# GlassyWing/yolo_deepsort

Measured on AMD Instinct MI355X. Metric: end-to-end frames/sec (detect+ReID+assoc), 608x608, higher is better.
Workload: dtype f16x3

## Files before the change

yolo_deepsort_amd/csrc/conv_block1.hip:

```cpp
#include "conv_common.h"

#include <algorithm>

namespace yds {

namespace {

constexpr int TH = 8, TW = 16;
constexpr int BM = TH * TW, BN = 64, WM = 4, WN = 2, NW = 8, NT = NW * 64;
constexpr int PR = TH + 2, PC = TW + 2, PPIX = PR * PC;
constexpr int CMID = 32, CIN = 64, GIN = CIN / 32;
constexpr int W3_BYTES = 9 * BN * 128, XP_BYTES = GIN * PPIX * 128, HP_BYTES = PPIX * 128;
constexpr int SMEM = W3_BYTES + XP_BYTES + HP_BYTES;
constexpr int XCHUNKS = GIN * PPIX * 8, XLOADS = (XCHUNKS + NT - 1) / NT;

struct PatchRows {
    int img, oy0, ox0, H, W;
    __device__ __forceinline__ int operator()(int row) const {
        const int oy = oy0 + row / TW, ox = ox0 + row % TW;
        return oy < H && ox < W ? (img * H + oy) * W + ox : -1;
    }
};

template <int ACT, bool HALF>
__global__ __launch_bounds__(NT, 1) void conv_block1_f16x3(ConvKernelArgs p2, ConvKernelArgs p3, int tiles_y, int tiles_x, int n_tiles) {
    fp16_saturate_on();
    extern __shared__ __attribute__((aligned(16))) char smem[];
    char *w3 = smem, *xp = smem + W3_BYTES, *hp = smem + W3_BYTES + XP_BYTES;
    const int tid = threadIdx.x, lane = tid & 63, wave = tid >> 6, wm = wave / WN, wn = wave % WN, kb = lane >> 5;
    const int H = p2.H, W = p2.W;

    for (int i = tid; i < 9 * BN * 8; i += NT) {
        const int row = i >> 3, pos = i & 7, tap = row / BN, co = row - tap * BN;
        const int c = pos ^ ((row >> 1) & 7);
        *reinterpret_cast<f32x4 *>(w3 + row * 128 + pos * 16) =
            *reinterpret_cast<const f32x4 *>(reinterpret_cast<const char *>(p3.w) + ((size_t)co * 9 + tap) * 128 + c * 16);
    }
    h8 w2h[4], w2l[4];
#pragma unroll
    for (int sb = 0; sb < 4; ++sb) {
        const char *g = reinterpret_cast<const char *>(p2.w) + ((size_t)(lane & 31) * GIN + (sb >> 1)) * 128;
        w2h[sb] = *reinterpret_cast<const h8 *>(g + (2 * (sb & 1) + kb) * 16);
        w2l[sb] = *reinterpret_cast<const h8 *>(g + 64 + (2 * (sb & 1) + kb) * 16);
    }
    float bias2[16];
#pragma unroll
    for (int e = 0; e < 16; ++e) bias2[e] = p2.bias[(e & 3) + 8 * (e >> 2) + 4 * kb] * A_SCALE;
    const int r = wm * 32 + (lane & 31), py = r / TW, px = r - py * TW;
    const int brow = wn * 32 + (lane & 31);

    const bool xs = p2.fmt_x == FMT_F16;
    f32x4 nxt[XLOADS];
    auto fetch = [&](int tl) {
        const int img = tl / (tiles_y * tiles_x), rem = tl - img * (tiles_y * tiles_x);
        const int iy0 = (rem / tiles_x) * TH - 1, ix0 = (rem % tiles_x) * TW - 1;
#pragma unroll
        for (int l = 0; l < XLOADS; ++l) {
            const int i = tid + l * NT, c = i & 7, row = i >> 3, g = row / PPIX, pr = row - g * PPIX;
            const int iy = iy0 + pr / PC, ix = ix0 + pr % PC;
            nxt[l] = f32x4{0.f, 0.f, 0.f, 0.f};
            if (i < XCHUNKS && tl < n_tiles && (unsigned)iy < (unsigned)H && (unsigned)ix < (unsigned)W && !(xs && c >= 4))
                nxt[l] = *reinterpret_cast<const f32x4 *>(reinterpret_cast<const char *>(p2.x + ((size_t)(img * H + iy) * W + ix) * p2.ldx) +
                                                          (xs ? (g * 4 + c) * 16 : g * 128 + c * 16));
        }
    };
    fetch(blockIdx.x);
    for (int tl = blockIdx.x; tl < n_tiles; tl += gridDim.x) {
        const int img = tl / (tiles_y * tiles_x), rem = tl - img * (tiles_y * tiles_x);
        const int oy0 = (rem / tiles_x) * TH, ox0 = (rem % tiles_x) * TW;
        __syncthreads();
#pragma unroll
        for (int l = 0; l < XLOADS; ++l) {
            const int i = tid + l * NT, c = i & 7, row = i >> 3;
            if (i < XCHUNKS) *reinterpret_cast<f32x4 *>(xp + row * 128 + ((c ^ ((row >> 1) & 7)) << 4)) = nxt[l];
        }
        __syncthreads();
        fetch(tl + gridDim.x);
        if (wave < (PPIX + 31) / 32) {
            const int pix = wave * 32 + (lane & 31), pr = min(pix, PPIX - 1);
            f32x16 c1, c2;
#pragma unroll
            for (int e = 0; e < 16; ++e) { c1[e] = 0.f; c2[e] = 0.f; }
#pragma unroll
            for (int sb = 0; sb < 4; ++sb) {
                const int row = (sb >> 1) * PPIX + pr, sw = (row >> 1) & 7;
                const char *ap = xp + row * 128;
                const h8 xh = *reinterpret_cast<const h8 *>(ap + (((2 * (sb & 1) + kb) ^ sw) << 4));
                c1 = __builtin_amdgcn_mfma_f32_32x32x16_f16(w2h[sb], xh, c1, 0, 0, 0);
                if (!HALF) {
                    const h8 xl = *reinterpret_cast<const h8 *>(ap + (((4 + 2 * (sb & 1) + kb) ^ sw) << 4));
                    c2 = __builtin_amdgcn_mfma_f32_32x32x16_f16(w2h[sb], xl, c2, 0, 0, 0);
                    c2 = __builtin_amdgcn_mfma_f32_32x32x16_f16(w2l[sb], xh, c2, 0, 0, 0);
                }
            }
            const int ry = pr / PC, rc = pr - ry * PC;
            const bool inside = (unsigned)(oy0 - 1 + ry) < (unsigned)H && (unsigned)(ox0 - 1 + rc) < (unsigned)W;
            const int sw = (pr >> 1) & 7;
            if (pix < PPIX) {
                if (inside) {
#pragma unroll
                    for (int g = 0; g < 4; ++g) {
                        float v[4];
#pragma unroll
                        for (int c = 0; c < 4; ++c) {
                            const int e = g * 4 + c;
                            const float os = (HALF ? c1[e] : c1[e] + c2[e] * (1.f / LO_SCALE)) + bias2[e];
                            v[c] = ACT == ACT_LEAKY ? fmaxf(os, os * 0.1f) : apply_act<ACT>(os * (1.f / A_SCALE)) * A_SCALE;
                        }
                        h16x4 hi, lo;
                        if (HALF) {
#pragma unroll
                            for (int c = 0; c < 4; ++c) hi[c] = (_Float16)v[c];
                        } else {
                            h16_encode4_scaled(v, hi, lo);
                        }
                        *reinterpret_cast<h16x4 *>(hp + pr * 128 + ((g ^ sw) << 4) + kb * 8) = hi;
                        if (!HALF) *reinterpret_cast<h16x4 *>(hp + pr * 128 + (((4 + g) ^ sw) << 4) + kb * 8) = lo;
                    }
                } else {
                    const h16x4 z = {(_Float16)0.f, (_Float16)0.f, (_Float16)0.f, (_Float16)0.f};
#pragma unroll
                    for (int g = 0; g < (HALF ? 4 : 8); ++g) *reinterpret_cast<h16x4 *>(hp + pr * 128 + ((g ^ sw) << 4) + kb * 8) = z;
                }
            }
        }
        __syncthreads();
        f32x16 acc1[1][1], acc2[1][1];
#pragma unroll
        for (int e = 0; e < 16; ++e) { acc1[0][0][e] = 0.f; acc2[0][0][e] = 0.f; }
#pragma unroll
        for (int t = 0; t < 9; ++t) {
            const int j = (py + t / 3) * PC + px + t % 3;
            const int jsw = (j >> 1) & 7, wrow = t * BN + brow, wsw = (wrow >> 1) & 7;
            const char *ap = hp + j * 128, *bp = w3 + wrow * 128;
#pragma unroll
            for (int s = 0; s < 2; ++s) {
                const h8 ah = *reinterpret_cast<const h8 *>(ap + (((2 * s + kb) ^ jsw) << 4));
                const h8 bh = *reinterpret_cast<const h8 *>(bp + (((2 * s + kb) ^ wsw) << 4));
                acc1[0][0] = __builtin_amdgcn_mfma_f32_32x32x16_f16(ah, bh, acc1[0][0], 0, 0, 0);
                if (!HALF) {
                    const h8 al = *reinterpret_cast<const h8 *>(ap + (((4 + 2 * s + kb) ^ jsw) << 4));
                    const h8 bl = *reinterpret_cast<const h8 *>(bp + (((4 + 2 * s + kb) ^ wsw) << 4));
                    acc2[0][0] = __builtin_amdgcn_mfma_f32_32x32x16_f16(ah, bl, acc2[0][0], 0, 0, 0);
                    acc2[0][0] = __builtin_amdgcn_mfma_f32_32x32x16_f16(al, bh, acc2[0][0], 0, 0, 0);
                }
            }
        }
#pragma unroll
        for (int e = 0; e < 16; ++e) acc1[0][0][e] = (HALF ? acc1[0][0][e] : acc1[0][0][e] + acc2[0][0][e] * (1.f / LO_SCALE)) * (1.f / A_SCALE);
        conv_epilogue_rows<BM, BN, WM, WN, ACT, RES_AFTER_ACT, 1, 1, NT, PatchRows, true>(p3, acc1, reinterpret_cast<float *>(xp),
                                                                                           PatchRows{img, oy0, ox0, H, W}, 0, tid);
    }
}

template <int ACT, bool HALF> void launch_inst(const ConvKernelArgs &k2, const ConvKernelArgs &k3, hipStream_t s) {
    static_assert(BM * (BN + 4) * 4 <= XP_BYTES, "whole-tile epilogue staging must fit the input patch");
    const int n_img = k2.M / (k2.H * k2.W);
    const int tiles_y = (k2.H + TH - 1) / TH, tiles_x = (k2.W + TW - 1) / TW, n_tiles = n_img * tiles_y * tiles_x;
    static bool attr_set = false;
    auto kern = conv_block1_f16x3<ACT, HALF>;
    if (!attr_set) {
        YDS_HIP(hipFuncSetAttribute(reinterpret_cast<const void *>(kern), hipFuncAttributeMaxDynamicSharedMemorySize, SMEM));
        attr_set = true;
    }
    hipLaunchKernelGGL(kern, dim3(std::min(n_tiles, 256)), dim3(NT), SMEM, s, k2, k3, tiles_y, tiles_x, n_tiles);
    YDS_HIP(hipGetLastError());
}

}

bool conv_block1_applicable(const ConvKernelArgs &k2, const ConvKernelArgs &k3) {
    return k2.Cin == CIN && k2.ksize == 1 && k2.stride == 1 && k2.Cout == CMID && k2.res_mode == RES_NONE && (k2.fmt_x == FMT_H16 || k2.fmt_x == FMT_F16) &&
           k3.Cin == CMID && k3.ksize == 3 && k3.stride == 1 && k3.pad == 1 && k3.Cout == BN && k3.res_mode == RES_AFTER_ACT &&
           k3.fmt_r == k2.fmt_x && k3.fmt_y == k2.fmt_x && k3.res == k2.x && k3.ldr == k2.ldx && k3.H == k2.H && k3.W == k2.W &&
           k2.act == k3.act && (k2.act == ACT_LEAKY || k2.act == ACT_MISH);
}

void launch_conv_block1(const ConvKernelArgs &k2, const ConvKernelArgs &k3, hipStream_t s) {
    if (!conv_block1_applicable(k2, k3)) fail("conv: the fused residual block takes conv1x1 64->32 + conv3x3 32->64 + shortcut to the block input");
    const bool half = k3.terms == 1;
    if (k2.act == ACT_LEAKY) { if (half) launch_inst<ACT_LEAKY, true>(k2, k3, s); else launch_inst<ACT_LEAKY, false>(k2, k3, s); }
    else { if (half) launch_inst<ACT_MISH, true>(k2, k3, s); else launch_inst<ACT_MISH, false>(k2, k3, s); }
}

}
```

yolo_deepsort_amd/csrc/conv_common.h:

```cpp
#pragma once
#include "common.h"
#include "h16.h"

#include <algorithm>
#include <stdlib.h>
#include <type_traits>

namespace yds {

typedef float f32x16 __attribute__((ext_vector_type(16)));
typedef float f32x4 __attribute__((ext_vector_type(4)));

typedef _Float16 h8 __attribute__((ext_vector_type(8)));
typedef _Float16 h4 __attribute__((ext_vector_type(4)));
constexpr float A_SCALE = 1.f / 256.f, LO_SCALE = 2048.f;
typedef __attribute__((address_space(3))) void lds_void_t;
typedef __attribute__((address_space(1))) const void glb_void_t;
template <int N> __device__ __forceinline__ void wait_vmcnt() { asm volatile("s_waitcnt vmcnt(%0)" ::"n"(N) : "memory"); }

struct ConvKernelArgs {
    const float *x, *w, *bias, *res;
    float *y;
    int H, W, Cin, ldx;
    int Ho, Wo, Cout, ldy, ldr;
    int ksize, stride, pad;
    int K, Kpad, M;
    int act, res_mode;
    int fmt_x, fmt_y, fmt_r;
    int terms;
    int ksplit = 1;
    float *y2 = nullptr;
    int ldy2 = 0, n_split = 0;
    int tiles_m, tiles_n, xm, rm, rn;
    int gn = 1;
    int gn_req = 0;
};

constexpr int KALIGN = 32;
constexpr int STAGGER = 24;

template <int ACT> __device__ __forceinline__ float apply_act(float v) {
    if (ACT == ACT_LEAKY) return v > 0.f ? v : v * 0.1f;
    if (ACT == ACT_RELU) return v > 0.f ? v : 0.f;
    if (ACT == ACT_MISH) {
        const float e = __builtin_amdgcn_exp2f(fminf(v, 20.f) * 1.44269504088896341f);
        const float n = e * (e + 2.f);
        const float m = v * (n * __builtin_amdgcn_rcpf(n + 2.f));
        return v > 20.f ? v : m;
    }
    return v;
}

__device__ __forceinline__ bool tile_of_block(const ConvKernelArgs &p, int &tm, int &tn) {
    const int b = blockIdx.x, xcd = b & 7, idx = b >> 3;
    int lm, ln;
    if (p.gn <= 1) {
        lm = idx % p.rm;
        ln = idx / p.rm;
    } else {
        const int per = p.rm * p.gn, grp = idx / per, w = idx - grp * per;
        const int g = min(p.gn, p.rn - grp * p.gn);
        lm = w / g;
        ln = grp * p.gn + (w - lm * g);
    }
    tm = (xcd % p.xm) * p.rm + lm;
    tn = (xcd / p.xm) * p.rn + ln;
    return tm < p.tiles_m && tn < p.tiles_n;
}

inline int plan_tile_map(ConvKernelArgs &k, int BM, int BN) {
    k.tiles_m = (k.M + BM - 1) / BM;
    k.tiles_n = (k.Cout + BN - 1) / BN;
    long best = -1;
    for (int xm = 1; xm <= 8; xm *= 2) {
        int xn = 8 / xm;
        int rm = (k.tiles_m + xm - 1) / xm, rn = (k.tiles_n + xn - 1) / xn;
        long waste = (long)rm * rn * 8 - (long)k.tiles_m * k.tiles_n;
        long cost = ((long)rm * BM + (long)rn * BN) * 64 + waste * (BM + BN);
        if (best < 0 || cost < best) { best = cost; k.xm = xm; k.rm = rm; k.rn = rn; }
    }
    k.gn = std::max(1, std::min(k.gn_req, k.rn));
    return 8 * k.rm * k.rn;
}

struct FlatRows {
    int m0;
    __device__ __forceinline__ int operator()(int row) const { return m0 + row; }
};
template <int BM, int BN, int WM, int WN, int ACT, int RES, int NT, class RowMap, bool ONE_PASS, class Store>
__device__ __forceinline__ void conv_epilogue_core(const ConvKernelArgs &p, Store store, float *stage, RowMap rows, int n0, int tid) {
    constexpr int ROWS = BM / WM, LD = BN + 4, C4 = BN / 4;
    constexpr int RSTEP = NT / C4;
    static_assert(NT % C4 == 0 && C4 % 2 == 0 && ROWS % RSTEP == 0, "tile width must divide the workgroup; lane pairs share a row");
    const int wave = tid >> 6, wm = wave / WN;
    const int c4 = tid % C4, rr = tid / C4;
    const int n = n0 + c4 * 4;
    const bool n_vec = n + 3 < p.Cout;
    const bool second = p.n_split > 0 && n >= p.n_split;
    float *const y_base = second ? p.y2 : p.y;
    const int y_ld = second ? p.ldy2 : p.ldy, ny = second ? n - p.n_split : n;
    float4 bias4 = make_float4(0.f, 0.f, 0.f, 0.f);
    if (n_vec) bias4 = *reinterpret_cast<const float4 *>(p.bias + n);
    else {
        if (n < p.Cout) bias4.x = p.bias[n];
        if (n + 1 < p.Cout) bias4.y = p.bias[n + 1];
        if (n + 2 < p.Cout) bias4.z = p.bias[n + 2];
    }
    constexpr int PER_PASS = ROWS / RSTEP, NRES = RES != RES_NONE ? WM * PER_PASS : 1;
    auto sweep = [&](auto yf_c, auto rf_c) {
        constexpr int YF = decltype(yf_c)::value, RF = decltype(rf_c)::value;
        constexpr bool YH = YF == FMT_H16, RH = RF == FMT_H16, YS = YF == FMT_F16, RS = RF == FMT_F16;
        float4 rraw[NRES];
        if (RES != RES_NONE) {
#pragma unroll
            for (int q = 0; q < NRES; ++q) {
                const int m = rows((q / PER_PASS) * ROWS + rr + (q % PER_PASS) * RSTEP);
                rraw[q] = make_float4(0.f, 0.f, 0.f, 0.f);
                if (m >= 0 && m < p.M && n < p.Cout) {
                    const float *rp = p.res + (size_t)m * p.ldr;
                    if (RH) {
                        const char *g = reinterpret_cast<const char *>(rp + (n & ~31)) + (n & 31) * 2;
                        const float2 hi = *reinterpret_cast<const float2 *>(g), lo = *reinterpret_cast<const float2 *>(g + 64);
                        rraw[q] = make_float4(hi.x, hi.y, lo.x, lo.y);
                    } else if (RS) {
                        const float2 h = *reinterpret_cast<const float2 *>(reinterpret_cast<const char *>(rp) + n * 2);
                        rraw[q] = make_float4(h.x, h.y, 0.f, 0.f);
                    } else if (n_vec) {
                        rraw[q] = *reinterpret_cast<const float4 *>(rp + n);
                    } else {
                        rraw[q].x = rp[n];
                        if (n + 1 < p.Cout) rraw[q].y = rp[n + 1];
                        if (n + 2 < p.Cout) rraw[q].z = rp[n + 2];
                    }
                }
            }
        }
#pragma unroll
        for (int pass = 0; pass < WM; ++pass) {
            if (ONE_PASS ? pass == 0 : wm == pass) store(stage + (ONE_PASS ? wm * ROWS * LD : 0));
            if (!ONE_PASS || pass == 0) __syncthreads();
#pragma unroll
            for (int k2 = 0; k2 < PER_PASS; ++k2) {
                const int r = rr + k2 * RSTEP;
                const int m = rows(pass * ROWS + r);
                const bool live = m >= 0 && m < p.M && n < p.Cout;
                float4 v = *reinterpret_cast<const float4 *>(stage + (ONE_PASS ? pass * ROWS * LD : 0) + r * LD + c4 * 4);
                float rs[4] = {0.f, 0.f, 0.f, 0.f};
                if (RES != RES_NONE) {
                    const float4 t = rraw[RES != RES_NONE ? pass * PER_PASS + k2 : 0];
                    if (RH) {
                        union { float2 f; h16x4 h; } uh, ul;
                        uh.f = make_float2(t.x, t.y);
                        ul.f = make_float2(t.z, t.w);
                        h16_decode4(uh.h, ul.h, rs);
                    } else if (RS) {
                        union { float2 f; h16x4 h; } uh;
                        uh.f = make_float2(t.x, t.y);
#pragma unroll
                        for (int k = 0; k < 4; ++k) rs[k] = (float)uh.h[k] * (1.f / H16_A_SCALE);
                    } else { rs[0] = t.x; rs[1] = t.y; rs[2] = t.z; rs[3] = t.w; }
                }
                float o[4] = {v.x + bias4.x, v.y + bias4.y, v.z + bias4.z, v.w + bias4.w};
#pragma unroll
                for (int k = 0; k < 4; ++k) {
                    if (RES == RES_BEFORE_ACT) o[k] += rs[k];
                    o[k] = apply_act<ACT>(o[k]);
                    if (RES == RES_AFTER_ACT) o[k] += rs[k];
                }
                float *yp = y_base + (size_t)m * y_ld;
                if (YH) {
                    h16x4 hi, lo;
                    h16_encode4(o, hi, lo);
                    const bool odd = c4 & 1;
                    union { h16x4 h; int i[2]; } send, recv;
                    send.h = odd ? hi : lo;
                    recv.i[0] = __builtin_amdgcn_update_dpp(send.i[0], send.i[0], 0xB1, 0xF, 0xF, false);
                    recv.i[1] = __builtin_amdgcn_update_dpp(send.i[1], send.i[1], 0xB1, 0xF, 0xF, false);
                    union { h16x4 h[2]; float4 f; } out;
                    out.h[0] = odd ? recv.h : hi;
                    out.h[1] = odd ? lo : recv.h;
                    const int nq = ny & ~7;
                    char *g = reinterpret_cast<char *>(yp + (nq & ~31)) + (nq & 31) * 2 + (odd ? 64 : 0);
                    if (live) *reinterpret_cast<float4 *>(g) = out.f;
                } else if (YS) {
                    union { h16x4 h; int i[2]; } mine, other;
#pragma unroll
                    for (int k = 0; k < 4; ++k) mine.h[k] = (_Float16)(o[k] * H16_A_SCALE);
                    other.i[0] = __builtin_amdgcn_update_dpp(mine.i[0], mine.i[0], 0xB1, 0xF, 0xF, false);
                    other.i[1] = __builtin_amdgcn_update_dpp(mine.i[1], mine.i[1], 0xB1, 0xF, 0xF, false);
                    union { h16x4 h[2]; float4 f; } out;
                    out.h[0] = mine.h;
                    out.h[1] = other.h;
                    if (live && !(c4 & 1)) *reinterpret_cast<float4 *>(reinterpret_cast<char *>(yp) + ny * 2) = out.f;
                } else if (live) {
                    if (n_vec) *reinterpret_cast<float4 *>(yp + ny) = make_float4(o[0], o[1], o[2], o[3]);
                    else { yp[ny] = o[0]; if (n + 1 < p.Cout) yp[ny + 1] = o[1]; if (n + 2 < p.Cout) yp[ny + 2] = o[2]; }
                }
            }
            if (!ONE_PASS && pass + 1 < WM) __syncthreads();
        }
    };
    using F32c = std::integral_constant<int, FMT_F32>;
    using H16c = std::integral_constant<int, FMT_H16>;
    using F16c = std::integral_constant<int, FMT_F16>;
    const bool yh = p.fmt_y == FMT_H16, rh = RES != RES_NONE && p.fmt_r == FMT_H16;
    if (p.fmt_y == FMT_F16) {
        sweep(F16c{}, F16c{});
    } else if (yh) {
        if (rh) sweep(H16c{}, H16c{});
        else sweep(H16c{}, F32c{});
    } else {
        if (rh) sweep(F32c{}, H16c{});
        else sweep(F32c{}, F32c{});
    }
}
constexpr size_t conv_stage_bytes(int BM, int BN) { return (size_t)BM * (BN + 4) * sizeof(float); }

template <int BM, int BN, int WM, int WN, int ACT, int RES, int TM, int TN, int NT = 256, class RowMap = FlatRows, bool ONE_PASS = false>
__device__ __forceinline__ void conv_epilogue_rows(const ConvKernelArgs &p, f32x16 (&acc)[TM][TN], float *stage, RowMap rows, int n0, int tid) {
    constexpr int LD = BN + 4;
    const int lane = tid & 63, wn = (tid >> 6) % WN;
    const int col = lane & 31, rsel = (lane >> 5) * 4;
    auto store = [&](float *st) {
#pragma unroll
        for (int i = 0; i < TM; ++i)
#pragma unroll
            for (int j = 0; j < TN; ++j)
#pragma unroll
                for (int e = 0; e < 16; ++e)
                    st[(i * 32 + rsel + (e & 3) + 8 * (e >> 2)) * LD + wn * (BN / WN) + j * 32 + col] = acc[i][j][e];
    };
    conv_epilogue_core<BM, BN, WM, WN, ACT, RES, NT, RowMap, ONE_PASS>(p, store, stage, rows, n0, tid);
}

template <int BM, int BN, int WM, int WN, int ACT, int RES, int TM, int TN, int NT = 256, class RowMap = FlatRows, bool ONE_PASS = false>
__device__ __forceinline__ void conv_epilogue16_rows(const ConvKernelArgs &p, f32x4 (&acc)[TM][TN], float *stage, RowMap rows, int n0, int tid) {
    constexpr int LD = BN + 4;
    const int lane = tid & 63, wn = (tid >> 6) % WN;
    const int col = lane & 15, rsel = (lane >> 4) * 4;
    auto store = [&](float *st) {
#pragma unroll
        for (int i = 0; i < TM; ++i)
#pragma unroll
            for (int j = 0; j < TN; ++j)
#pragma unroll
                for (int e = 0; e < 4; ++e)
                    st[(i * 16 + rsel + e) * LD + wn * (BN / WN) + j * 16 + col] = acc[i][j][e];
    };
    conv_epilogue_core<BM, BN, WM, WN, ACT, RES, NT, RowMap, ONE_PASS>(p, store, stage, rows, n0, tid);
}
template <int BM, int BN, int WM, int WN, int ACT, int RES, int TM, int TN, int NT = 256, bool ONE_PASS = false>
__device__ __forceinline__ void conv_epilogue16(const ConvKernelArgs &p, f32x4 (&acc)[TM][TN], float *stage, int m0, int n0, int tid) {
    conv_epilogue16_rows<BM, BN, WM, WN, ACT, RES, TM, TN, NT, FlatRows, ONE_PASS>(p, acc, stage, FlatRows{m0}, n0, tid);
}

template <int BM, int BN, int WM, int WN, int ACT, int RES, int TM, int TN, int NT = 256, bool ONE_PASS = false>
__device__ __forceinline__ void conv_epilogue(const ConvKernelArgs &p, f32x16 (&acc)[TM][TN], float *stage, int m0, int n0, int tid) {
    conv_epilogue_rows<BM, BN, WM, WN, ACT, RES, TM, TN, NT, FlatRows, ONE_PASS>(p, acc, stage, FlatRows{m0}, n0, tid);
}

ConvKernelArgs make_conv_args(const ConvArgs &a);
bool conv_stem2_applicable(const ConvKernelArgs &k0, const ConvKernelArgs &k1);
void launch_conv_stem2(const ConvKernelArgs &k0, const ConvKernelArgs &k1, hipStream_t s);
bool conv_block1_applicable(const ConvKernelArgs &k2, const ConvKernelArgs &k3);
void launch_conv_block1(const ConvKernelArgs &k2, const ConvKernelArgs &k3, hipStream_t s);

template <class F> void dispatch_act_res(const ConvKernelArgs &k, F f) {
    using Linear = std::integral_constant<int, ACT_LINEAR>;
    using Leaky = std::integral_constant<int, ACT_LEAKY>;
    using Mish = std::integral_constant<int, ACT_MISH>;
    using Relu = std::integral_constant<int, ACT_RELU>;
    using None = std::integral_constant<int, RES_NONE>;
    using After = std::integral_constant<int, RES_AFTER_ACT>;
    using Before = std::integral_constant<int, RES_BEFORE_ACT>;
    switch (k.act * 4 + k.res_mode) {
        case ACT_LINEAR * 4 + RES_NONE: f(Linear{}, None{}); break;
        case ACT_LEAKY * 4 + RES_NONE: f(Leaky{}, None{}); break;
        case ACT_LEAKY * 4 + RES_AFTER_ACT: f(Leaky{}, After{}); break;
        case ACT_MISH * 4 + RES_NONE: f(Mish{}, None{}); break;
        case ACT_MISH * 4 + RES_AFTER_ACT: f(Mish{}, After{}); break;
        case ACT_RELU * 4 + RES_NONE: f(Relu{}, None{}); break;
        case ACT_RELU * 4 + RES_BEFORE_ACT: f(Relu{}, Before{}); break;
        default: fail("conv: unsupported activation/residual combination (%d, %d)", k.act, k.res_mode);
    }
}

template <auto KERN, class... Args>
void launch_conv_tiles(ConvKernelArgs k, int BM, int BN, int grid_y, int threads, size_t smem, hipStream_t s, Args... args) {
    static size_t attr_set = 0;
    if (smem > attr_set) {
        YDS_HIP(hipFuncSetAttribute(reinterpret_cast<const void *>(KERN), hipFuncAttributeMaxDynamicSharedMemorySize, (int)smem));
        attr_set = smem;
    }
    dim3 grid(plan_tile_map(k, BM, BN), grid_y);
    hipLaunchKernelGGL(KERN, grid, dim3(threads), smem, s, k, args...);
    YDS_HIP(hipGetLastError());
}

bool conv_direct_applicable(const ConvKernelArgs &k);
void launch_conv_direct(const ConvKernelArgs &k, hipStream_t s);
bool conv_pool_applicable(const ConvKernelArgs &k);
void launch_conv_pool(const ConvKernelArgs &k, hipStream_t s);

void launch_conv_f16x3_staged(ConvKernelArgs k, int tile, hipStream_t s);
void launch_conv_f16x3_dma(ConvKernelArgs k, int tile, hipStream_t s);
void launch_conv_f16x3_win(ConvKernelArgs k, int tile, hipStream_t s);
void launch_conv_f16x3_splitk(ConvKernelArgs k, int tile, hipStream_t s);
bool conv_splitk_applicable(const ConvKernelArgs &k, int tile);
bool conv_splitk_preferred(const ConvKernelArgs &k);
bool conv_win2_applicable(const ConvKernelArgs &k);
void launch_conv_win2(ConvKernelArgs k, hipStream_t s);
bool conv_win_applicable(const ConvKernelArgs &k);
void launch_conv_win(ConvKernelArgs k, int shape, hipStream_t s);
void conv_win_clock(unsigned long long *cycles_ticks, bool reset);
void conv_win16_clock(unsigned long long *cycles_ticks, bool reset);
bool conv_win16_small_applicable(const ConvKernelArgs &k);
void launch_conv_win16(ConvKernelArgs k, int shape, hipStream_t s);
void conv_win2_clock(unsigned long long *cycles_ticks, bool reset);

}
```

yolo_deepsort_amd/csrc/conv_stem2.hip:

```cpp
#include "conv_common.h"

#include <algorithm>


namespace yds {

namespace {

typedef float f32x2 __attribute__((ext_vector_type(2)));

constexpr int TH = 8, TW = 16;
constexpr int BM = TH * TW, BN = 64, WM = 4, WN = 2, NW = 8, NT = NW * 64;
constexpr int PR = 2 * TH + 1, PC = 2 * TW + 1;
constexpr int EVEN_COLS = TW + 1, ODD_COLS = TW;
constexpr int ODD_BASE = PR * EVEN_COLS;
constexpr int PATCH_ROWS = PR * PC;
constexpr int RR = PR + 2, RC = PC + 2;
constexpr int W_BYTES = 9 * BN * 128, PATCH_BYTES = PATCH_ROWS * 128, RGB_BYTES = RR * RC * 16;
constexpr int SMEM = W_BYTES + PATCH_BYTES + RGB_BYTES;

struct StemRows {
    int img, oy0, ox0, Ho, Wo;
    __device__ __forceinline__ int operator()(int row) const {
        const int oy = oy0 + row / TW, ox = ox0 + row % TW;
        return oy < Ho && ox < Wo ? (img * Ho + oy) * Wo + ox : -1;
    }
};

__device__ __forceinline__ int patch_row(int ry, int rc) {
    return (rc & 1) ? ODD_BASE + ry * ODD_COLS + (rc >> 1) : ry * EVEN_COLS + (rc >> 1);
}

template <int ACT0, int ACT1, bool HALF>
__global__ __launch_bounds__(NT, 1) void conv_stem2_f16x3(ConvKernelArgs p0, ConvKernelArgs p1, int tiles_y, int tiles_x, int n_tiles) {
    fp16_saturate_on();
    extern __shared__ __attribute__((aligned(16))) char smem[];
    char *wreg = smem, *patch = smem + W_BYTES;
    float4 *rgb = reinterpret_cast<float4 *>(smem + W_BYTES + PATCH_BYTES);
    const int tid = threadIdx.x, lane = tid & 63, wave = tid >> 6, wm = wave / WN, wn = wave % WN;

    for (int i = tid; i < 9 * BN * 8; i += NT) {
        const int row = i >> 3, pos = i & 7, tap = row / BN, co = row - tap * BN;
        const int c = pos ^ ((row >> 1) & 7);
        const f32x4 v = *reinterpret_cast<const f32x4 *>(reinterpret_cast<const char *>(p1.w) + ((size_t)min(co, p1.Cout - 1) * 9 + tap) * 128 + c * 16);
        *reinterpret_cast<f32x4 *>(wreg + row * 128 + pos * 16) = v;
    }
    const int kb0 = lane >> 5;
    h8 w0h[3], w0l[3];
#pragma unroll
    for (int sb = 0; sb < 3; ++sb)
#pragma unroll
        for (int e = 0; e < 8; ++e) {
            const int t = 4 * sb + 2 * kb0 + (e >> 2), c = e & 3;
            const float x = (t < 9 && c < 3) ? p0.w[(size_t)(lane & 31) * p0.Kpad + t * 4 + c] : (t == 4 && c == 3 ? p0.bias[lane & 31] : 0.f);
            const _Float16 h = (_Float16)x;
            w0h[sb][e] = h;
            w0l[sb][e] = (_Float16)((x - (float)h) * LO_SCALE);
        }
    const int kb = lane >> 5, r = wm * 32 + (lane & 31), py = r / TW, px = r - py * TW;
    const int brow = wn * 32 + (lane & 31);

    constexpr int LOADS = (RR * RC + NT - 1) / NT;
    float4 nxt[LOADS];
    auto fetch = [&](int tl) {
        const int img = tl / (tiles_y * tiles_x), rem = tl - img * (tiles_y * tiles_x);
        const int iy0 = 2 * ((rem / tiles_x) * TH) - 2, ix0 = 2 * ((rem % tiles_x) * TW) - 2;
#pragma unroll
        for (int l = 0; l < LOADS; ++l) {
            const int i = tid + l * NT, rr = i / RC, cc = i - rr * RC;
            const int iy = iy0 + rr, ix = ix0 + cc;
            nxt[l] = make_float4(0.f, 0.f, 0.f, 0.f);
            if (i < RR * RC && tl < n_tiles && (unsigned)iy < (unsigned)p0.H && (unsigned)ix < (unsigned)p0.W) {
                nxt[l] = *reinterpret_cast<const float4 *>(p0.x + ((size_t)(img * p0.H + iy) * p0.W + ix) * p0.ldx);
                nxt[l].w = 1.f;
            }
        }
    };
    fetch(blockIdx.x);
    for (int tl = blockIdx.x; tl < n_tiles; tl += gridDim.x) {
        const int img = tl / (tiles_y * tiles_x), rem = tl - img * (tiles_y * tiles_x);
        const int oy0 = (rem / tiles_x) * TH, ox0 = (rem % tiles_x) * TW;
        const int ly0 = 2 * oy0 - 1, lx0 = 2 * ox0 - 1;
        __syncthreads();
#pragma unroll
        for (int l = 0; l < LOADS; ++l) {
            const int i = tid + l * NT;
            if (i < RR * RC) {
                const float v[4] = {nxt[l].x, nxt[l].y, nxt[l].z, nxt[l].w};
                union { h16x4 h[2]; float4 f; } sp;
                h16_encode4(v, sp.h[0], sp.h[1]);
                rgb[i] = sp.f;
            }
        }
        __syncthreads();
        fetch(tl + gridDim.x);
#pragma unroll 1
        for (int fr = wave; fr < (PATCH_ROWS + 31) / 32; fr += NW) {
            const int pix = fr * 32 + (lane & 31), pc = min(pix, PATCH_ROWS - 1);
            const int ry = pc / PC, rc = pc - ry * PC;
            f32x16 c1, c2;
#pragma unroll
            for (int e = 0; e < 16; ++e) { c1[e] = 0.f; c2[e] = 0.f; }
#pragma unroll
            for (int sb = 0; sb < 3; ++sb) {
                union { h16x4 q[2]; h8 v; } xh, xl;
#pragma unroll
                for (int u = 0; u < 2; ++u) {
                    const int t = 4 * sb + 2 * kb0 + u;
                    union { float4 f; h16x4 h[2]; } px4;
                    px4.f = make_float4(0.f, 0.f, 0.f, 0.f);
                    if (t < 9) px4.f = rgb[(ry + t / 3) * RC + rc + t % 3];
                    xh.q[u] = px4.h[0];
                    xl.q[u] = px4.h[1];
                }
                c1 = __builtin_amdgcn_mfma_f32_32x32x16_f16(w0h[sb], xh.v, c1, 0, 0, 0);
                if (!HALF) {
                    c2 = __builtin_amdgcn_mfma_f32_32x32x16_f16(w0h[sb], xl.v, c2, 0, 0, 0);
                    c2 = __builtin_amdgcn_mfma_f32_32x32x16_f16(w0l[sb], xh.v, c2, 0, 0, 0);
                }
            }
            const bool inside = (unsigned)(ly0 + ry) < (unsigned)p0.H && (unsigned)(lx0 + rc) < (unsigned)p0.W;
            const int j = patch_row(ry, rc), jsw = (j >> 1) & 7;
            if (pix < PATCH_ROWS) {
                if (inside) {
#pragma unroll
                    for (int g = 0; g < 4; ++g) {
                        float v[4];
#pragma unroll
                        for (int c = 0; c < 4; ++c) {
                            const int e = g * 4 + c;
                            const float os = HALF ? c1[e] : c1[e] + c2[e] * (1.f / LO_SCALE);
                            v[c] = ACT0 == ACT_LEAKY ? fmaxf(os, os * 0.1f) : apply_act<ACT0>(os * (1.f / A_SCALE)) * A_SCALE;
                        }
                        h16x4 hi, lo;
                        if (HALF) {
#pragma unroll
                            for (int c = 0; c < 4; ++c) hi[c] = (_Float16)v[c];
                        } else {
                            h16_encode4_scaled(v, hi, lo);
                        }
                        *reinterpret_cast<h16x4 *>(patch + j * 128 + ((g ^ jsw) << 4) + kb0 * 8) = hi;
                        if (!HALF) *reinterpret_cast<h16x4 *>(patch + j * 128 + (((4 + g) ^ jsw) << 4) + kb0 * 8) = lo;
                    }
                } else {
                    const h16x4 z = {(_Float16)0.f, (_Float16)0.f, (_Float16)0.f, (_Float16)0.f};
#pragma unroll
                    for (int g = 0; g < (HALF ? 4 : 8); ++g) *reinterpret_cast<h16x4 *>(patch + j * 128 + ((g ^ jsw) << 4) + kb0 * 8) = z;
                }
            }
        }
        __syncthreads();
        f32x16 acc1[1][1], acc2[1][1];
#pragma unroll
        for (int e = 0; e < 16; ++e) { acc1[0][0][e] = 0.f; acc2[0][0][e] = 0.f; }
#pragma unroll
        for (int t = 0; t < 9; ++t) {
            const int dy = t / 3, dx = t % 3;
            const int j = (dx & 1) ? ODD_BASE + (2 * py + dy) * ODD_COLS + px : (2 * py + dy) * EVEN_COLS + px + (dx >> 1);
            const int jsw = (j >> 1) & 7, wrow = t * BN + brow, wsw = (wrow >> 1) & 7;
            const char *ap = patch + j * 128, *bp = wreg + wrow * 128;
#pragma unroll
            for (int s = 0; s < 2; ++s) {
                const h8 ah = *reinterpret_cast<const h8 *>(ap + (((2 * s + kb) ^ jsw) << 4));
                const h8 bh = *reinterpret_cast<const h8 *>(bp + (((2 * s + kb) ^ wsw) << 4));
                acc1[0][0] = __builtin_amdgcn_mfma_f32_32x32x16_f16(ah, bh, acc1[0][0], 0, 0, 0);
                if (!HALF) {
                    const h8 al = *reinterpret_cast<const h8 *>(ap + (((4 + 2 * s + kb) ^ jsw) << 4));
                    const h8 bl = *reinterpret_cast<const h8 *>(bp + (((4 + 2 * s + kb) ^ wsw) << 4));
                    acc2[0][0] = __builtin_amdgcn_mfma_f32_32x32x16_f16(ah, bl, acc2[0][0], 0, 0, 0);
                    acc2[0][0] = __builtin_amdgcn_mfma_f32_32x32x16_f16(al, bh, acc2[0][0], 0, 0, 0);
                }
            }
        }
#pragma unroll
        for (int e = 0; e < 16; ++e) acc1[0][0][e] = (HALF ? acc1[0][0][e] : acc1[0][0][e] + acc2[0][0][e] * (1.f / LO_SCALE)) * (1.f / A_SCALE);
        __syncthreads();
        conv_epilogue_rows<BM, BN, WM, WN, ACT1, RES_NONE, 1, 1, NT, StemRows, true>(p1, acc1, reinterpret_cast<float *>(patch),
                                                                                       StemRows{img, oy0, ox0, p1.Ho, p1.Wo}, 0, tid);
    }
}

template <int ACT0, int ACT1, bool HALF> void launch_inst(const ConvKernelArgs &k0, const ConvKernelArgs &k1, hipStream_t s) {
    static_assert(BM * (BN + 4) * 4 <= PATCH_BYTES, "whole-tile epilogue staging must fit the layer-0 patch");
    const int n_img = k0.M / (k0.H * k0.W);
    const int tiles_y = (k1.Ho + TH - 1) / TH, tiles_x = (k1.Wo + TW - 1) / TW, n_tiles = n_img * tiles_y * tiles_x;
    static bool attr_set = false;
    auto kern = conv_stem2_f16x3<ACT0, ACT1, HALF>;
    if (!attr_set) {
        YDS_HIP(hipFuncSetAttribute(reinterpret_cast<const void *>(kern), hipFuncAttributeMaxDynamicSharedMemorySize, SMEM));
        attr_set = true;
    }
    hipLaunchKernelGGL(kern, dim3(std::min(n_tiles, 256)), dim3(NT), SMEM, s, k0, k1, tiles_y, tiles_x, n_tiles);
    YDS_HIP(hipGetLastError());
}

}

bool conv_stem2_applicable(const ConvKernelArgs &k0, const ConvKernelArgs &k1) {
    return k0.Cin == 4 && k0.ksize == 3 && k0.stride == 1 && k0.pad == 1 && k0.Cout == 32 && k0.res_mode == RES_NONE && k0.fmt_x == FMT_F32 &&
           k1.Cin == 32 && k1.ksize == 3 && k1.stride == 2 && k1.pad == 1 && k1.Cout == 64 && k1.res_mode == RES_NONE && k1.K == 288 &&
           k1.H == k0.Ho && k1.W == k0.Wo && k0.act == k1.act && (k0.act == ACT_LEAKY || k0.act == ACT_MISH);
}

void launch_conv_stem2(const ConvKernelArgs &k0, const ConvKernelArgs &k1, hipStream_t s) {
    if (!conv_stem2_applicable(k0, k1)) fail("conv: the fused stem takes a 3x3/s1 RGB->32 conv followed by a 3x3/s2 32->64 conv");
    const bool half = k1.terms == 1;
    if (k0.act == ACT_LEAKY) { if (half) launch_inst<ACT_LEAKY, ACT_LEAKY, true>(k0, k1, s); else launch_inst<ACT_LEAKY, ACT_LEAKY, false>(k0, k1, s); }
    else { if (half) launch_inst<ACT_MISH, ACT_MISH, true>(k0, k1, s); else launch_inst<ACT_MISH, ACT_MISH, false>(k0, k1, s); }
}

}
```

yolo_deepsort_amd/csrc/h16.h:

```cpp
#pragma once
#include <hip/hip_runtime.h>

namespace yds {

enum TensorFmt { FMT_F32 = 0, FMT_H16 = 1, FMT_F16 = 2 };
__host__ __device__ inline int fmt_slots(int fmt, int c) { return fmt == FMT_F16 ? c / 2 : c; }

constexpr float H16_A_SCALE = 1.f / 256.f, H16_LO_SCALE = 2048.f;

typedef _Float16 h16x4 __attribute__((ext_vector_type(4)));

__device__ __forceinline__ void fp16_saturate_on() { asm volatile("s_setreg_imm32_b32 hwreg(HW_REG_MODE, 23, 1), 1"); }

__device__ __forceinline__ void h16_encode4(const float v[4], h16x4 &hi, h16x4 &lo) {
#pragma unroll
    for (int c = 0; c < 4; ++c) {
        float xs = v[c] * H16_A_SCALE;
        _Float16 h = (_Float16)xs;
        hi[c] = h;
        lo[c] = (_Float16)((xs - (float)h) * H16_LO_SCALE);
    }
}

__device__ __forceinline__ void h16_encode4_scaled(const float xs[4], h16x4 &hi, h16x4 &lo) {
#pragma unroll
    for (int c = 0; c < 4; ++c) {
        _Float16 h = (_Float16)xs[c];
        hi[c] = h;
        lo[c] = (_Float16)((xs[c] - (float)h) * H16_LO_SCALE);
    }
}

__device__ __forceinline__ void h16_decode4(const h16x4 &hi, const h16x4 &lo, float v[4]) {
#pragma unroll
    for (int c = 0; c < 4; ++c) v[c] = ((float)hi[c] + (float)lo[c] * (1.f / H16_LO_SCALE)) * (1.f / H16_A_SCALE);
}

__device__ __forceinline__ void h16_load4(const float *pixel, int c, float v[4]) {
    const char *g = reinterpret_cast<const char *>(pixel + (c & ~31)) + (c & 31) * 2;
    h16x4 hi = *reinterpret_cast<const h16x4 *>(g), lo = *reinterpret_cast<const h16x4 *>(g + 64);
    h16_decode4(hi, lo, v);
}
__device__ __forceinline__ void h16_store4(float *pixel, int c, const float v[4]) {
    char *g = reinterpret_cast<char *>(pixel + (c & ~31)) + (c & 31) * 2;
    h16x4 hi, lo;
    h16_encode4(v, hi, lo);
    *reinterpret_cast<h16x4 *>(g) = hi;
    *reinterpret_cast<h16x4 *>(g + 64) = lo;
}

__device__ __forceinline__ void f16_load4(const float *pixel, int c, float v[4]) {
    const h16x4 h = *reinterpret_cast<const h16x4 *>(reinterpret_cast<const char *>(pixel) + c * 2);
#pragma unroll
    for (int k = 0; k < 4; ++k) v[k] = (float)h[k] * (1.f / H16_A_SCALE);
}
__device__ __forceinline__ void f16_store4(float *pixel, int c, const float v[4]) {
    h16x4 h;
#pragma unroll
    for (int k = 0; k < 4; ++k) h[k] = (_Float16)(v[k] * H16_A_SCALE);
    *reinterpret_cast<h16x4 *>(reinterpret_cast<char *>(pixel) + c * 2) = h;
}

__device__ __forceinline__ void load4(const float *pixel, int c, int fmt, float v[4]) {
    if (fmt == FMT_H16) h16_load4(pixel, c, v);
    else if (fmt == FMT_F16) f16_load4(pixel, c, v);
    else {
        float4 t = *reinterpret_cast<const float4 *>(pixel + c);
        v[0] = t.x; v[1] = t.y; v[2] = t.z; v[3] = t.w;
    }
}
__device__ __forceinline__ void store4(float *pixel, int c, int fmt, const float v[4]) {
    if (fmt == FMT_H16) h16_store4(pixel, c, v);
    else if (fmt == FMT_F16) f16_store4(pixel, c, v);
    else *reinterpret_cast<float4 *>(pixel + c) = make_float4(v[0], v[1], v[2], v[3]);
}

}
```

Measured before the change: 1701.

## Interleave LDS reads with MFMAs and streamline f16x3 encode and stem RGB layout

Adds a sched_group_barrier helper that interleaves LDS reads between MFMA instructions in the 3x3 loops of the block1 and stem2 kernels, so shared-memory latency can hide behind matrix math. The f16x3 hi/lo combine becomes a single FMA, and the scaled encoder uses inline v_fma_mix instructions to cut conversion instruction count. In stem2 the RGB staging buffer is split into separate hi and lo planes with a zero slot, and per-fragment index math is precomputed and unrolled. This raises register pressure, and the hand-written asm and scheduling hints depend on the compiler following them.

```diff
diff --git a/yolo_deepsort_amd/csrc/conv_block1.hip b/yolo_deepsort_amd/csrc/conv_block1.hip
--- a/yolo_deepsort_amd/csrc/conv_block1.hip
+++ b/yolo_deepsort_amd/csrc/conv_block1.hip
@@ -104,7 +104,7 @@
 #pragma unroll
                         for (int c = 0; c < 4; ++c) {
                             const int e = g * 4 + c;
-                            const float os = (HALF ? c1[e] : c1[e] + c2[e] * (1.f / LO_SCALE)) + bias2[e];
+                            const float os = (HALF ? c1[e] : f16x3_sum(c1[e], c2[e])) + bias2[e];
                             v[c] = ACT == ACT_LEAKY ? fmaxf(os, os * 0.1f) : apply_act<ACT>(os * (1.f / A_SCALE)) * A_SCALE;
                         }
                         h16x4 hi, lo;
@@ -146,8 +146,9 @@
                 }
             }
         }
+        sched_reads_under_mfmas<18, HALF ? 2 : 4, HALF ? 1 : 3>();
 #pragma unroll
-        for (int e = 0; e < 16; ++e) acc1[0][0][e] = (HALF ? acc1[0][0][e] : acc1[0][0][e] + acc2[0][0][e] * (1.f / LO_SCALE)) * (1.f / A_SCALE);
+        for (int e = 0; e < 16; ++e) acc1[0][0][e] = (HALF ? acc1[0][0][e] : f16x3_sum(acc1[0][0][e], acc2[0][0][e])) * (1.f / A_SCALE);
         conv_epilogue_rows<BM, BN, WM, WN, ACT, RES_AFTER_ACT, 1, 1, NT, PatchRows, true>(p3, acc1, reinterpret_cast<float *>(xp),
                                                                                            PatchRows{img, oy0, ox0, H, W}, 0, tid);
     }
diff --git a/yolo_deepsort_amd/csrc/conv_common.h b/yolo_deepsort_amd/csrc/conv_common.h
--- a/yolo_deepsort_amd/csrc/conv_common.h
+++ b/yolo_deepsort_amd/csrc/conv_common.h
@@ -14,6 +14,22 @@
 typedef _Float16 h8 __attribute__((ext_vector_type(8)));
 typedef _Float16 h4 __attribute__((ext_vector_type(4)));
 constexpr float A_SCALE = 1.f / 256.f, LO_SCALE = 2048.f;
+__device__ __forceinline__ float f16x3_sum(float c1, float c2) { return __builtin_fmaf(c2, 1.f / LO_SCALE, c1); }
+template <int STEPS, int READS, int MFMAS> __device__ __forceinline__ void sched_reads_under_mfmas() {
+    static_assert(READS % 2 == 0 && (MFMAS == 1 || MFMAS == 3), "two reads per slot");
+    __builtin_amdgcn_sched_group_barrier(0x100, READS, 0);
+#pragma unroll
+    for (int i = 0; i + 1 < STEPS; ++i) {
+        __builtin_amdgcn_sched_group_barrier(0x008, 1, 0);
+        __builtin_amdgcn_sched_group_barrier(0x100, MFMAS == 1 ? READS : READS / 2, 0);
+        if (MFMAS == 3) {
+            __builtin_amdgcn_sched_group_barrier(0x008, 1, 0);
+            __builtin_amdgcn_sched_group_barrier(0x100, READS / 2, 0);
+            __builtin_amdgcn_sched_group_barrier(0x008, 1, 0);
+        }
+    }
+    __builtin_amdgcn_sched_group_barrier(0x008, MFMAS, 0);
+}
 typedef __attribute__((address_space(3))) void lds_void_t;
 typedef __attribute__((address_space(1))) const void glb_void_t;
 template <int N> __device__ __forceinline__ void wait_vmcnt() { asm volatile("s_waitcnt vmcnt(%0)" ::"n"(N) : "memory"); }
diff --git a/yolo_deepsort_amd/csrc/conv_stem2.hip b/yolo_deepsort_amd/csrc/conv_stem2.hip
--- a/yolo_deepsort_amd/csrc/conv_stem2.hip
+++ b/yolo_deepsort_amd/csrc/conv_stem2.hip
@@ -16,7 +16,9 @@
 constexpr int ODD_BASE = PR * EVEN_COLS;
 constexpr int PATCH_ROWS = PR * PC;
 constexpr int RR = PR + 2, RC = PC + 2;
-constexpr int W_BYTES = 9 * BN * 128, PATCH_BYTES = PATCH_ROWS * 128, RGB_BYTES = RR * RC * 16;
+constexpr int NFRAG = (PATCH_ROWS + 31) / 32, NFR = (NFRAG + NW - 1) / NW;
+constexpr int RGB_ZERO = RR * RC * 8, RGB_LO = RGB_ZERO + 8, RGB_BYTES = 2 * RGB_LO;
+constexpr int W_BYTES = 9 * BN * 128, PATCH_BYTES = PATCH_ROWS * 128;
 constexpr int SMEM = W_BYTES + PATCH_BYTES + RGB_BYTES;
 
 struct StemRows {
@@ -36,7 +38,7 @@
     fp16_saturate_on();
     extern __shared__ __attribute__((aligned(16))) char smem[];
     char *wreg = smem, *patch = smem + W_BYTES;
-    float4 *rgb = reinterpret_cast<float4 *>(smem + W_BYTES + PATCH_BYTES);
+    char *rgb = smem + W_BYTES + PATCH_BYTES;
     const int tid = threadIdx.x, lane = tid & 63, wave = tid >> 6, wm = wave / WN, wn = wave % WN;
 
     for (int i = tid; i < 9 * BN * 8; i += NT) {
@@ -57,6 +59,23 @@
             w0h[sb][e] = h;
             w0l[sb][e] = (_Float16)((x - (float)h) * LO_SCALE);
         }
+    int fbase[NFR], fst[NFR], fsw[NFR], fry[NFR], frc[NFR], toff[5];
+#pragma unroll
+    for (int k = 0; k < NFR; ++k) {
+        const int pix = (wave + k * NW) * 32 + (lane & 31), pc = min(pix, PATCH_ROWS - 1);
+        fry[k] = pc / PC;
+        frc[k] = pc - fry[k] * PC;
+        fbase[k] = (fry[k] * RC + frc[k]) * 8;
+        const int j = patch_row(fry[k], frc[k]);
+        fst[k] = pix < PATCH_ROWS ? j * 128 + kb0 * 8 : -1;
+        fsw[k] = ((j >> 1) & 7) << 4;
+    }
+#pragma unroll
+    for (int q = 0; q < 5; ++q) {
+        const int t = min(4 * (q >> 1) + 2 * kb0 + (q & 1), 8);
+        toff[q] = ((t / 3) * RC + t % 3) * 8;
+    }
+    if (tid < 2) *reinterpret_cast<h16x4 *>(rgb + RGB_ZERO + tid * RGB_LO) = h16x4{(_Float16)0.f, (_Float16)0.f, (_Float16)0.f, (_Float16)0.f};
     const int kb = lane >> 5, r = wm * 32 + (lane & 31), py = r / TW, px = r - py * TW;
     const int brow = wn * 32 + (lane & 31);
 
@@ -87,17 +106,17 @@
             const int i = tid + l * NT;
             if (i < RR * RC) {
                 const float v[4] = {nxt[l].x, nxt[l].y, nxt[l].z, nxt[l].w};
-                union { h16x4 h[2]; float4 f; } sp;
-                h16_encode4(v, sp.h[0], sp.h[1]);
-                rgb[i] = sp.f;
+                h16x4 hi, lo;
+                h16_encode4(v, hi, lo);
+                *reinterpret_cast<h16x4 *>(rgb + i * 8) = hi;
+                *reinterpret_cast<h16x4 *>(rgb + RGB_LO + i * 8) = lo;
             }
         }
         __syncthreads();
         fetch(tl + gridDim.x);
-#pragma unroll 1
-        for (int fr = wave; fr < (PATCH_ROWS + 31) / 32; fr += NW) {
-            const int pix = fr * 32 + (lane & 31), pc = min(pix, PATCH_ROWS - 1);
-            const int ry = pc / PC, rc = pc - ry * PC;
+#pragma unroll
+        for (int k = 0; k < NFR; ++k) {
+            if ((k + 1) * NW > NFRAG && wave + k * NW >= NFRAG) continue;
             f32x16 c1, c2;
 #pragma unroll
             for (int e = 0; e < 16; ++e) { c1[e] = 0.f; c2[e] = 0.f; }
@@ -106,12 +125,13 @@
                 union { h16x4 q[2]; h8 v; } xh, xl;
 #pragma unroll
                 for (int u = 0; u < 2; ++u) {
-                    const int t = 4 * sb + 2 * kb0 + u;
-                    union { float4 f; h16x4 h[2]; } px4;
-                    px4.f = make_float4(0.f, 0.f, 0.f, 0.f);
-                    if (t < 9) px4.f = rgb[(ry + t / 3) * RC + rc + t % 3];
-                    xh.q[u] = px4.h[0];
-                    xl.q[u] = px4.h[1];
+                    xh.q[u] = xl.q[u] = h16x4{(_Float16)0.f, (_Float16)0.f, (_Float16)0.f, (_Float16)0.f};
+                    if (4 * sb + u < 9) {
+                        int a = fbase[k] + toff[2 * sb + u];
+                        if (4 * sb + u + 2 >= 9) a = kb0 ? RGB_ZERO : a;
+                        xh.q[u] = *reinterpret_cast<const h16x4 *>(rgb + a);
+                        if (!HALF) xl.q[u] = *reinterpret_cast<const h16x4 *>(rgb + RGB_LO + a);
+                    }
                 }
                 c1 = __builtin_amdgcn_mfma_f32_32x32x16_f16(w0h[sb], xh.v, c1, 0, 0, 0);
                 if (!HALF) {
@@ -119,9 +139,10 @@
                     c2 = __builtin_amdgcn_mfma_f32_32x32x16_f16(w0l[sb], xh.v, c2, 0, 0, 0);
                 }
             }
-            const bool inside = (unsigned)(ly0 + ry) < (unsigned)p0.H && (unsigned)(lx0 + rc) < (unsigned)p0.W;
-            const int j = patch_row(ry, rc), jsw = (j >> 1) & 7;
-            if (pix < PATCH_ROWS) {
+            const bool inside = (unsigned)(ly0 + fry[k]) < (unsigned)p0.H && (unsigned)(lx0 + frc[k]) < (unsigned)p0.W;
+            char *row = patch + fst[k];
+            const int jsw = fsw[k];
+            if (fst[k] >= 0) {
                 if (inside) {
 #pragma unroll
                     for (int g = 0; g < 4; ++g) {
@@ -129,7 +150,7 @@
 #pragma unroll
                         for (int c = 0; c < 4; ++c) {
                             const int e = g * 4 + c;
-                            const float os = HALF ? c1[e] : c1[e] + c2[e] * (1.f / LO_SCALE);
+                            const float os = HALF ? c1[e] : f16x3_sum(c1[e], c2[e]);
                             v[c] = ACT0 == ACT_LEAKY ? fmaxf(os, os * 0.1f) : apply_act<ACT0>(os * (1.f / A_SCALE)) * A_SCALE;
                         }
                         h16x4 hi, lo;
@@ -139,13 +160,13 @@
                         } else {
                             h16_encode4_scaled(v, hi, lo);
                         }
-                        *reinterpret_cast<h16x4 *>(patch + j * 128 + ((g ^ jsw) << 4) + kb0 * 8) = hi;
-                        if (!HALF) *reinterpret_cast<h16x4 *>(patch + j * 128 + (((4 + g) ^ jsw) << 4) + kb0 * 8) = lo;
+                        *reinterpret_cast<h16x4 *>(row + ((g << 4) ^ jsw)) = hi;
+                        if (!HALF) *reinterpret_cast<h16x4 *>(row + (((4 + g) << 4) ^ jsw)) = lo;
                     }
                 } else {
                     const h16x4 z = {(_Float16)0.f, (_Float16)0.f, (_Float16)0.f, (_Float16)0.f};
 #pragma unroll
-                    for (int g = 0; g < (HALF ? 4 : 8); ++g) *reinterpret_cast<h16x4 *>(patch + j * 128 + ((g ^ jsw) << 4) + kb0 * 8) = z;
+                    for (int g = 0; g < (HALF ? 4 : 8); ++g) *reinterpret_cast<h16x4 *>(row + ((g << 4) ^ jsw)) = z;
                 }
             }
         }
@@ -172,8 +193,9 @@
                 }
             }
         }
-#pragma unroll
-        for (int e = 0; e < 16; ++e) acc1[0][0][e] = (HALF ? acc1[0][0][e] : acc1[0][0][e] + acc2[0][0][e] * (1.f / LO_SCALE)) * (1.f / A_SCALE);
+        sched_reads_under_mfmas<18, HALF ? 2 : 4, HALF ? 1 : 3>();
+#pragma unroll
+        for (int e = 0; e < 16; ++e) acc1[0][0][e] = (HALF ? acc1[0][0][e] : f16x3_sum(acc1[0][0][e], acc2[0][0][e])) * (1.f / A_SCALE);
         __syncthreads();
         conv_epilogue_rows<BM, BN, WM, WN, ACT1, RES_NONE, 1, 1, NT, StemRows, true>(p1, acc1, reinterpret_cast<float *>(patch),
                                                                                        StemRows{img, oy0, ox0, p1.Ho, p1.Wo}, 0, tid);
diff --git a/yolo_deepsort_amd/csrc/h16.h b/yolo_deepsort_amd/csrc/h16.h
--- a/yolo_deepsort_amd/csrc/h16.h
+++ b/yolo_deepsort_amd/csrc/h16.h
@@ -23,12 +23,21 @@
 }
 
 __device__ __forceinline__ void h16_encode4_scaled(const float xs[4], h16x4 &hi, h16x4 &lo) {
+    union { h16x4 h; int i[2]; } uh, ul;
 #pragma unroll
-    for (int c = 0; c < 4; ++c) {
-        _Float16 h = (_Float16)xs[c];
-        hi[c] = h;
-        lo[c] = (_Float16)((xs[c] - (float)h) * H16_LO_SCALE);
+    for (int c = 0; c < 4; ++c) uh.h[c] = (_Float16)xs[c];
+    float d[4];
+#pragma unroll
+    for (int c = 0; c < 4; c += 2) {
+        asm("v_fma_mix_f32 %0, %1, -1.0, %2 op_sel_hi:[1,0,0]" : "=v"(d[c]) : "v"(uh.i[c >> 1]), "v"(xs[c]));
+        asm("v_fma_mix_f32 %0, %1, -1.0, %2 op_sel:[1,0,0] op_sel_hi:[1,0,0]" : "=v"(d[c + 1]) : "v"(uh.i[c >> 1]), "v"(xs[c + 1]));
     }
+    asm("v_fma_mixlo_f16 %0, %1, %2, 0" : "=v"(ul.i[0]) : "v"(d[0]), "s"(H16_LO_SCALE));
+    asm("v_fma_mixlo_f16 %0, %1, %2, 0" : "=v"(ul.i[1]) : "v"(d[2]), "s"(H16_LO_SCALE));
+    asm("v_fma_mixhi_f16 %0, %1, %2, 0" : "+v"(ul.i[0]) : "v"(d[1]), "s"(H16_LO_SCALE));
+    asm("v_fma_mixhi_f16 %0, %1, %2, 0" : "+v"(ul.i[1]) : "v"(d[3]), "s"(H16_LO_SCALE));
+    hi = uh.h;
+    lo = ul.h;
 }
 
 __device__ __forceinline__ void h16_decode4(const h16x4 &hi, const h16x4 &lo, float v[4]) {
```

After: 1707, median of 6. Within noise of the previous version (+0.4%).
